# Belis0811/MaskUnet

Hardware: AMD Instinct MI355X
Metric: 128x128 images/sec (fwd+bwd) (higher is better)
Workload: dtype f16; 1 GPU; ADE20K-semantic shape 128x128, c_out=150, batch=64/GPU, 1-head MaskAttn-UNet fwd+bwd, train mode; global_batch=64, parallelism=dp1, mask_mode=fixed, loss=maskunet_amd.CrossEntropyLoss on module output, optimizer_in_step=False, hip_graph=False

## Files before the change

include/maskunet_hip.h:

```cpp
#ifndef MASKUNET_HIP_H
#define MASKUNET_HIP_H

#ifdef __cplusplus
extern "C" {
#endif

#define MU_OK 0
#define MU_ERR_ARG (-1)
#define MU_ERR_SHAPE (-2)
#define MU_ERR_LAUNCH (-3)
#define MU_ERR_WORKSPACE (-4)

#define MU_F32 0
#define MU_F16 1
#define MU_F32X 2

#define MU_ACT_NONE 0
#define MU_ACT_GELU 1
#define MU_ACT_RELU 2

const char* mu_version_host(void);

int mu_transpose(const void* src, int src_dtype, long src_ld, void* dst, int dst_dtype, long dst_ld, int batch, int R, int C,
                 void* stream);
// ... 51 lines not shown

long mu_bn_workspace_bytes(int C);
int mu_bn_train_stats(const void* x, long M, int C, long ld, float* mean, float* rstd, float* running_mean, float* running_var,
                      long* num_batches_tracked, int c_valid, float momentum, float eps, void* workspace, long ws_bytes, int dtype,
                      void* stream);
int mu_bn_train_stats_rows(const float* stat_part, int rows, long M, int C, float* mean, float* rstd, float* running_mean,
                           float* running_var, long* num_batches_tracked, int c_valid, float momentum, float eps, void* workspace,
                           long ws_bytes, void* stream);
int mu_bn_eval_stats(const float* running_mean, const float* running_var, float eps, float* mean, float* rstd, int C, int c_valid,
                     void* stream);
int mu_bn_eval_fold(const float* running_mean1, const float* running_var1, const float* gamma1, const float* beta1, float eps1,
                    const float* running_mean2, const float* running_var2, const float* gamma2, const float* beta2, float eps2,
                    const float* conv_bias, float* scale, float* shift, int C, int c_valid, void* stream);
int mu_bn_act_fwd(const void* x, const void* res, void* y, long M, int C, long ld, const float* mean, const float* rstd,
                  const float* gamma, const float* beta, int act, int dtype, void* stream);
int mu_bn_act_fwd_enc(const void* x, const void* res, void* y_enc, void* y16, long M, int C, const float* mean, const float* rstd,
                      const float* gamma, const float* beta, int act, void* stream);
int mu_bn_act_bwd(const void* x, const void* res, const void* grad_out, void* dx, void* dres, long M, int C, long ld,
                  const float* mean, const float* rstd, const float* gamma, const float* beta, int act, int training, float* dgamma,
                  float* dbeta, void* workspace, long ws_bytes, int dtype, void* stream);
int mu_bn_pair_compose(const float* rstd1, const float* gamma1, const float* beta1, const float* gamma2, int C, int c_valid, long M,
                       float eps1, float eps2, float momentum2, float* running_mean2, float* running_var2,
                       long* num_batches_tracked2, float* gamma_eff, float* xhat_scale, float* dgamma2_coef, float* dgamma1_coef,
                       void* stream);
int mu_bn_act_bwd_scaled(const void* x, const void* res, const void* grad_out, void* dx, void* dres, long M, int C, long ld,
                         const float* mean, const float* rstd, const float* gamma, const float* beta, int act, int training,
                         float* dgamma, float* dbeta, const float* xhat_scale, void* workspace, long ws_bytes, int dtype, void* stream);

int mu_bn_pair_bwd(const void* x, const void* grad_out, void* dx, long M, int C, long ld, const float* mean, const float* rstd,
                   const float* gamma_eff, const float* beta2, const float* xhat_scale, const float* dgamma2_coef,
                   const float* dgamma1_coef, float* pair_grads, float* dbeta2, void* workspace, long ws_bytes, int dtype, void* stream);

int mu_bn_act_bwd_h(const void* x, const void* res, const void* grad_out, void* dx_h, void* dres, long M, int C, const float* mean,
                    const float* rstd, const float* gamma, const float* beta, int act, int training, float* dgamma, float* dbeta,
                    float* dy_scale, void* workspace, long ws_bytes, void* stream);
int mu_bn_pair_bwd_h(const void* x, const void* grad_out, void* dx_h, long M, int C, const float* mean, const float* rstd,
                     const float* gamma_eff, const float* beta2, const float* xhat_scale, const float* dgamma2_coef,
                     const float* dgamma1_coef, float* pair_grads, float* dbeta2, float* dy_scale, void* workspace, long ws_bytes,
                     void* stream);

long mu_ln_sample_workspace_bytes(int B);
int mu_ln_sample_fwd(const void* x, const float* w, const float* b, void* y, float* mean, float* rstd, int B, long L, float eps,
                     void* workspace, long ws_bytes, int dtype, void* stream);
int mu_ln_sample_bwd(const void* x, const void* dy, const float* w, const float* mean, const float* rstd, void* dx, float* dw,
                     float* db, int B, long L, void* workspace, long ws_bytes, int dtype, void* stream);

int mu_maxpool2_fwd(const void* x, void* y, int B, int H, int W, int C, int dtype, void* stream);
int mu_maxpool2_bwd(const void* x, const void* dy, void* dx, int B, int H, int W, int C, int dtype, void* stream);
int mu_maxpool2_bwd_acc(const void* x, const void* dy, const void* dy2, const void* dx_add, void* dx, int B, int H, int W, int C, int dtype,
                        void* stream);
int mu_upcat_fwd(const void* x, const void* skip, void* y, int B, int h, int w, int Cx, int Cs, int dtype, void* stream);
int mu_upcat_bwd(const void* dy, void* dx, void* dskip, int B, int h, int w, int Cx, int Cs, int dtype, void* stream);
int mu_upcat_bwd_acc(const void* dy, const void* dy2, void* dx, void* dskip, int B, int h, int w, int Cx, int Cs, int dtype, void* stream);
int mu_upcat_compact_fwd(const void* x, const void* skip, void* y, int B, int h, int w, int Cx_ld, int Cx_valid, int Cs_ld, int Cs_valid,
                         int Ct_ld, int dtype, void* stream);
int mu_upcat_compact_bwd(const void* dy, void* dx, void* dskip, int B, int h, int w, int Cx_ld, int Cx_valid, int Cs_ld, int Cs_valid,
                         int Ct_ld, int dtype, void* stream);
int mu_dropout(const void* x, void* y, long n, float p, unsigned long long seed, const unsigned char* mask, unsigned char* mask_out,
               int dtype, void* stream);
int mu_dropout_step(const void* x, void* y, long n, float p, unsigned long long seed, const unsigned long long* seed_step,
// ... 145 lines not shown
```

maskunet_amd/_lib.py:

```python
from __future__ import annotations

import ctypes
import os
from ctypes import c_char_p, c_float, c_int, c_long, c_ulonglong, c_void_p

import torch

_HERE = os.path.dirname(os.path.abspath(__file__))
LIB_PATH = os.environ.get("MU_LIB_PATH") or os.path.join(_HERE, "libmaskunet_hip.so")

MU_F32, MU_F16, MU_F32X = 0, 1, 2
ACT_NONE, ACT_GELU, ACT_RELU = 0, 1, 2
MU_IDMAP_I32, MU_IDMAP_I64, MU_IDMAP_RGB8 = 0, 1, 2
_ERR = {-1: "MU_ERR_ARG", -2: "MU_ERR_SHAPE", -3: "MU_ERR_LAUNCH", -4: "MU_ERR_WORKSPACE"}

P, I, L, F = c_void_p, c_int, c_long, c_float
SIGNATURES = {
    "mu_version_host": (c_char_p, []),
    "mu_transpose": (I, [P, I, L, P, I, L, I, I, I, P]),
    "mu_transpose_pad": (I, [P, I, L, P, I, L, I, I, I, I, P]),
    "mu_cast": (I, [P, I, P, I, L, P]),
    "mu_split_encode": (I, [P, P, L, P]),
    "mu_split_encode_h": (I, [P, P, L, P]),
    "mu_split_encode_h4": (I, [P, P, L, P]),
# ... 25 lines not shown
    "mu_conv_wgrad_bias": (I, [P, P, P, P, I, I, I, I, I, I, I, I, L, L, P, L, I, P]),
    "mu_colsum_workspace_bytes": (L, [I]),
    "mu_colsum": (I, [P, L, I, L, P, P, L, I, P]),
    "mu_bn_workspace_bytes": (L, [I]),
    "mu_bn_train_stats": (I, [P, L, I, L, P, P, P, P, P, I, F, F, P, L, I, P]),
    "mu_bn_train_stats_rows": (I, [P, I, L, I, P, P, P, P, P, I, F, F, P, L, P]),
    "mu_bn_eval_stats": (I, [P, P, F, P, P, I, I, P]),
    "mu_bn_act_fwd": (I, [P, P, P, L, I, L, P, P, P, P, I, I, P]),
    "mu_bn_act_bwd": (I, [P, P, P, P, P, L, I, L, P, P, P, P, I, I, P, P, P, L, I, P]),
    "mu_bn_pair_compose": (I, [P, P, P, P, I, I, L, F, F, F, P, P, P, P, P, P, P, P]),
    "mu_bn_act_bwd_scaled": (I, [P, P, P, P, P, L, I, L, P, P, P, P, I, I, P, P, P, P, L, I, P]),
    "mu_bn_pair_bwd": (I, [P, P, P, L, I, L, P, P, P, P, P, P, P, P, P, P, L, I, P]),
    "mu_ln_sample_workspace_bytes": (L, [I]),
    "mu_ln_sample_fwd": (I, [P, P, P, P, P, P, I, L, F, P, L, I, P]),
    "mu_ln_sample_bwd": (I, [P, P, P, P, P, P, P, P, I, L, P, L, I, P]),
    "mu_maxpool2_fwd": (I, [P, P, I, I, I, I, I, P]),
    "mu_maxpool2_bwd": (I, [P, P, P, I, I, I, I, I, P]),
    "mu_upcat_fwd": (I, [P, P, P, I, I, I, I, I, I, P]),
    "mu_upcat_bwd": (I, [P, P, P, I, I, I, I, I, I, P]),
    "mu_upcat_compact_fwd": (I, [P, P, P, I, I, I, I, I, I, I, I, I, P]),
    "mu_upcat_compact_bwd": (I, [P, P, P, I, I, I, I, I, I, I, I, I, P]),
    "mu_dropout": (I, [P, P, L, F, c_ulonglong, P, P, I, P]),
    "mu_dropout_step": (I, [P, P, L, F, c_ulonglong, P, P, P, I, P]),
    "mu_add": (I, [P, P, P, L, I, P]),
    "mu_attn_fwd": (I, [P, P, P, P, P, P, P, P, P, P, P, I, I, I, I, F, I, P]),
    "mu_attn_bwd_workspace_bytes": (L, [I, I, I]),
    "mu_attn_bwd": (I, [P, P, P, P, P, P, P, P, P, P, P, P, P, P, P, I, I, I, I, P, L, I, P]),
    "mu_gather_rows": (I, [P, L, P, P, P, I, I, I, P]),
    "mu_scatter_rows": (I, [P, P, P, P, L, I, I, I, P]),
    "mu_softmax_rows": (I, [P, I, I, P, F, I, P]),
# ... 180 lines not shown
```

maskunet_amd/csrc/norm.hip:

```cpp
#include "common.h"
#include "../../include/maskunet_hip.h"

#define MU_STAT_MAXBLK 1024

template <typename T, int MODE, int ACT = -1, int RES = -1, bool MAXT = false>
__global__ __launch_bounds__(256, 1) void bn_partial_kernel(const T* __restrict__ x, const T* __restrict__ g, const T* __restrict__ res,
                                                         T* __restrict__ dzbuf, long M, int C, long ld,
                                                         const float* __restrict__ mean, const float* __restrict__ rstd,
                                                         const float* __restrict__ gamma, const float* __restrict__ beta, int act_arg,
                                                         double* __restrict__ part, float* __restrict__ pmax = nullptr) {
    constexpr int N = Vec16<T>::N;
    constexpr int U = MODE == 0 ? 8 : 2;
    constexpr bool FAST = sizeof(T) == 2;
    const int act = ACT >= 0 ? ACT : act_arg;
    const bool has_res = RES >= 0 ? (RES != 0) : (res != nullptr);
    extern __shared__ __attribute__((aligned(16))) double sh[];
    const int cv = C / N;
    const int rpi = 256 / cv;
    const int tc = threadIdx.x % cv, tr = threadIdx.x / cv;
    const long r0 = (long)blockIdx.x * (U * rpi), r1 = M;
    const long rstride = (long)gridDim.x * (U * rpi);
    double s0[N], s1[N];
    float mxg[N], mxx[N];
#pragma unroll
// ... 181 lines not shown
    if (lane) return;
    dbeta[c] = (float)a;
    dgamma[c] = (float)b;
    if (pair_grads) {
        pair_grads[c] = pc2[c] * (float)b;
        pair_grads[C + c] = pc1[c] * (float)b;
        pair_grads[2 * C + c] = 0.f;
    }
    const float s1c = training ? (float)(a / (double)M) : 0.f;
    const float s2c = training ? (float)((xscale ? (double)xscale[c] : 1.0) * b / (double)M) : 0.f;
    s1[c] = s1c;
    s2[c] = s2c;
    if (bound) bound[c] = fabsf(gamma[c] * rstd[c]) * (mg + fabsf(s1c) + mx * fabsf(s2c));
}

template <typename T, bool ENC = false, int ACT = -1, int RES = -1>
__global__ __launch_bounds__(256) void bn_act_fwd_kernel(const T* __restrict__ x, const T* __restrict__ res, T* __restrict__ y, long M,
                                                         int C, long ld, const float* __restrict__ mean, const float* __restrict__ rstd,
                                                         const float* __restrict__ gamma, const float* __restrict__ beta, int act_arg,
                                                         h16* __restrict__ y16 = nullptr) {
    constexpr int N = Vec16<T>::N;
    constexpr int U = 2;
    constexpr bool FAST = sizeof(T) == 2;
    const int act = ACT >= 0 ? ACT : act_arg;
    const bool has_res = RES >= 0 ? (RES != 0) : (res != nullptr);
    const int cv = C / N;
    const long total = M * cv;
    const long stride = (long)gridDim.x * 256;
    const long first = (long)blockIdx.x * 256 + threadIdx.x;
    const int c = (int)(first % cv) * N;
    const long rstep = stride / cv;
    float a[N], b[N];
#pragma unroll
    for (int i = 0; i < N; ++i) {
        a[i] = rstd[c + i] * gamma[c + i];
        b[i] = beta[c + i] - mean[c + i] * a[i];
    }
    for (long idx = first; idx < total; idx += U * stride) {
        const long r = idx / cv;
        Vec16<T> xv[U], rv[U];
#pragma unroll
        for (int u = 0; u < U; ++u) {
            if (idx + u * stride < total) {
                xv[u].load_nt(x + (r + u * rstep) * ld + c);
                if (has_res) rv[u].load_nt(res + (r + u * rstep) * ld + c);
            }
        }
#pragma unroll
        for (int u = 0; u < U; ++u) {
            if (idx + u * stride < total) {
                Vec16<T> o;
#pragma unroll
                for (int i = 0; i < N; i += 2) {
                    mu_f32x2 pp = __builtin_elementwise_fma(mu_f32x2{xv[u].get(i), xv[u].get(i + 1)}, mu_f32x2{a[i], a[i + 1]}, mu_f32x2{b[i], b[i + 1]});
                    if (has_res) pp += mu_f32x2{rv[u].get(i), rv[u].get(i + 1)};
                    float o0, o1;
                    mu_act2_t<FAST>(pp[0], pp[1], act, o0, o1);
                    o.set(i, o0);
                    o.set(i + 1, o1);
                }
                if constexpr (ENC) {
                    float o0 = o.get(0), o1 = o.get(1), o2 = o.get(2), o3 = o.get(3);
                    asm("" : "+v"(o0), "+v"(o1), "+v"(o2), "+v"(o3));
                    const uint4 e4 = mu_ench4((f32x4){o0, o1, o2, o3});
                    *reinterpret_cast<uint4*>(y + (r + u * rstep) * ld + c) = e4;
                    if (y16) *reinterpret_cast<uint2*>(y16 + (r + u * rstep) * (long)C + c) = make_uint2(e4.x, e4.y);
                } else {
                    o.store(y + (r + u * rstep) * ld + c);
                }
            }
        }
    }
}

template <typename T, bool RECOMP, bool ENC = false, int ACT = -1>
__global__ __launch_bounds__(256) void bn_bwd_apply_kernel(const T* __restrict__ x, const T* dzbuf, T* dx, long M, int C, long ld,
                                                           const float* __restrict__ mean, const float* __restrict__ rstd,
                                                           const float* __restrict__ gamma, const float* __restrict__ beta, int act_arg,
                                                           const float* __restrict__ s1, const float* __restrict__ s2,
                                                           const float* __restrict__ bound = nullptr, float* __restrict__ dy_scale = nullptr) {
    constexpr int N = Vec16<T>::N;
    constexpr int U = 2;
    constexpr bool FAST = sizeof(T) == 2;
    const int act = ACT >= 0 ? ACT : act_arg;
    const int cv = C / N;
    const long total = M * cv;
// ... 299 lines not shown
}

extern "C" int mu_bn_act_fwd(const void* x, const void* res, void* y, long M, int C, long ld, const float* mean, const float* rstd,
                             const float* gamma, const float* beta, int act, int dtype, void* stream) {
    if (!x || !y || !mean || !rstd || !gamma || !beta || M <= 0 || C <= 0 || C % 8 || ld < C) return MU_ERR_ARG;
    hipStream_t st = (hipStream_t)stream;
    if (act != MU_ACT_NONE && act != MU_ACT_GELU && act != MU_ACT_RELU) return MU_ERR_ARG;
    if (dtype == MU_F32X)
        return bn_act_fwd_launch<float, true>((const float*)x, (const float*)res, (float*)y, M, C, ld, mean, rstd, gamma, beta, act, st);
    return with_storage(dtype, [&](auto tag) -> int {
        using T = decltype(tag);
        return bn_act_fwd_launch<T, false>((const T*)x, (const T*)res, (T*)y, M, C, ld, mean, rstd, gamma, beta, act, st);
    });
}

template <typename T>
struct BnBwd {
    const T *x, *res, *g;
    T *dx, *dres;
    long M; int C; long ld;
    const float *mean, *rstd, *gamma, *beta;
    int act, training;
    float *dgamma, *dbeta;
    const float* xscale = nullptr;
    const float *pc2 = nullptr, *pc1 = nullptr;
    float* pair_grads = nullptr;
    float* dy_scale = nullptr;
};

template <typename T, bool ENC>
// ... 180 lines not shown
    double a = 0.0, c = 0.0;
    for (int k = lane; k < nchunk; k += 64) { a += part[((long)b * nchunk + k) * 2]; c += part[((long)b * nchunk + k) * 2 + 1]; }
    a = wave_sum_d(a); c = wave_sum_d(c);
    if (lane) return;
    if (mode == 0) {
        double m = a / (double)L, var = c / (double)L - m * m;
        if (var < 0.0) var = 0.0;
        o0[b] = (float)m;
        o1[b] = (float)(1.0 / sqrt(var + (double)eps));
    } else {
        o0[b] = (float)(a / (double)L);
        o1[b] = (float)(c / (double)L);
    }
}

template <typename T>
__global__ __launch_bounds__(256) void lns_fwd_apply_kernel(const T* __restrict__ x, const float* __restrict__ w, const float* __restrict__ bias,
                                                            const float* __restrict__ mean, const float* __restrict__ rstd, T* __restrict__ y,
                                                            long L, int B) {
    constexpr int N = Vec16<T>::N;
    const long nvec = L / N;
    for (long v = (long)blockIdx.x * 256 + threadIdx.x; v < nvec; v += (long)gridDim.x * 256) {
        float wv[N], bv[N];
#pragma unroll
        for (int i = 0; i < N; ++i) { wv[i] = w[v * N + i]; bv[i] = bias[v * N + i]; }
        for (int b = 0; b < B; ++b) {
            const float mu = mean[b], rs = rstd[b];
            Vec16<T> xv, o;
            xv.load_nt(x + (long)b * L + v * N);
#pragma unroll
            for (int i = 0; i < N; ++i) o.set(i, (xv.get(i) - mu) * rs * wv[i] + bv[i]);
            o.store(y + (long)b * L + v * N);
        }
    }
}

template <typename T>
__global__ __launch_bounds__(256) void lns_bwd_apply_kernel(const T* __restrict__ x, const T* __restrict__ dy, const float* __restrict__ w,
                                                            const float* __restrict__ mean, const float* __restrict__ rstd,
                                                            const float* __restrict__ m1, const float* __restrict__ m2, T* __restrict__ dx,
                                                            float* __restrict__ dw, float* __restrict__ db, long L, int B) {
    constexpr int N = Vec16<T>::N;
    const long nvec = L / N;
    for (long v = (long)blockIdx.x * 256 + threadIdx.x; v < nvec; v += (long)gridDim.x * 256) {
        float wv[N], aw[N], ab[N];
#pragma unroll
        for (int i = 0; i < N; ++i) { wv[i] = w[v * N + i]; aw[i] = 0.f; ab[i] = 0.f; }
        for (int b = 0; b < B; ++b) {
// ... 33 lines not shown
                                float eps, void* workspace, long ws_bytes, int dtype, void* stream) {
    if (!x || !w || !b || !y || !mean || !rstd || !workspace || B <= 0 || L <= 0 || L % 8) return MU_ERR_ARG;
    if (ws_bytes < LnWs::bytes(B)) return MU_ERR_WORKSPACE;
    hipStream_t st = (hipStream_t)stream;
    const LnWs ws(workspace, B);
    return with_storage(dtype, [&](auto tag) -> int {
        using T = decltype(tag);
        lns_partial_kernel<T, 0><<<dim3(LN_CHUNKS, B), 256, 0, st>>>((const T*)x, nullptr, nullptr, nullptr, nullptr, L, ws.part);
        lns_final_kernel<<<mu_cdiv(B, 4), 256, 0, st>>>(ws.part, LN_CHUNKS, L, eps, 0, mean, rstd, B);
        lns_fwd_apply_kernel<T><<<lns_apply_grid(L, Vec16<T>::N), 256, 0, st>>>((const T*)x, w, b, mean, rstd, (T*)y, L, B);
        MU_CHECK_LAUNCH();
        return MU_OK;
    });
}

extern "C" int mu_ln_sample_bwd(const void* x, const void* dy, const float* w, const float* mean, const float* rstd, void* dx,
                                float* dw, float* db, int B, long L, void* workspace, long ws_bytes, int dtype, void* stream) {
    if (!x || !dy || !w || !mean || !rstd || !dx || !dw || !db || !workspace || B <= 0 || L <= 0 || L % 8) return MU_ERR_ARG;
    if (ws_bytes < LnWs::bytes(B)) return MU_ERR_WORKSPACE;
    hipStream_t st = (hipStream_t)stream;
    const LnWs ws(workspace, B);
    return with_storage(dtype, [&](auto tag) -> int {
        using T = decltype(tag);
        lns_partial_kernel<T, 1><<<dim3(LN_CHUNKS, B), 256, 0, st>>>((const T*)x, (const T*)dy, w, mean, rstd, L, ws.part);
        lns_final_kernel<<<mu_cdiv(B, 4), 256, 0, st>>>(ws.part, LN_CHUNKS, L, 0.f, 1, ws.m1, ws.m2, B);
        lns_bwd_apply_kernel<T><<<lns_apply_grid(L, Vec16<T>::N), 256, 0, st>>>((const T*)x, (const T*)dy, w, mean, rstd, ws.m1, ws.m2, (T*)dx, dw, db, L, B);
        MU_CHECK_LAUNCH();
        return MU_OK;
    });
}
// ... 1 lines not shown
```

maskunet_amd/modules.py:

```python
from __future__ import annotations

import torch
import torch.nn as nn

from . import ops
from ._lib import ACT_GELU, ACT_NONE, ACT_RELU

_DEFAULT_DTYPE = torch.float32


def set_default_compute_dtype(dtype):
    global _DEFAULT_DTYPE
    if dtype not in (torch.float32, torch.float16):
        raise TypeError("compute dtype must be torch.float32 or torch.float16")
    _DEFAULT_DTYPE = dtype


class _HipModule(nn.Module):
    def __init__(self):
        super().__init__()
        self.compute_dtype = _DEFAULT_DTYPE

    def set_compute_dtype(self, dtype):
        if dtype not in (torch.float32, torch.float16):
# ... 167 lines not shown
    def forward_nhwc(self, x, skip_x, cx=None, cs=None, skip_link=None):
        link = ops.grad_link(x, skip_x)
        x = ops.upcat(x, skip_x, cx, cs, link, skip_link)
        return _conv_blocks(x, [self.conv[0], self.conv[1]], self.conv[2], link)

    def forward(self, x, skip_x):
        self._check_device(x)
        y = self.forward_nhwc(ops.to_nhwc(x, self.compute_dtype), ops.to_nhwc(skip_x, self.compute_dtype), x.shape[1], skip_x.shape[1])
        return ops.to_nchw(y, self.out_channels, x.dtype)


class _Head(nn.Sequential):
    """Conv2d 1x1 (bias) -> BatchNorm2d -> ReLU container with the reference's Sequential indices."""


def _head_1x1_bn_relu(seq, x):
    if ops.eval_fusable(seq[1]):
        return ops.conv_bn_act_eval(x, seq[0].weight, seq[0].bias, seq[1], ACT_RELU)
    y = ops.conv(x, seq[0].weight, seq[0].bias)
    return ops.bn_act(y, seq[1], ACT_RELU)


class UNet(_HipModule):

    def __init__(self, c_in=3, c_out=3, embed_dim=None, *, hw=128):
        super().__init__()
        self.c_out = c_out
        self.initial_conv = ConvBlock(c_in, 64)
        self.downsample1 = DownSample(64, 128)
        self.self_attention1 = Mask2FormerAttention(128, 128)
        self.downsample2 = DownSample(128, 256)
        self.self_attention2 = Mask2FormerAttention(256, 256)
        self.downsample3 = DownSample(256, 256)
        self.self_attention3 = Mask2FormerAttention(256, 256)

# ... 24 lines not shown

    def set_keep_masks(self, keeps):
        for blk, k in zip(self.attention_blocks(), keeps):
            blk.set_keep_mask(k)

    def set_mask_mode(self, mode):
        if mode not in ("fixed", "resample"):
            raise ValueError("mask_mode must be 'fixed' or 'resample'")
        for blk in self.attention_blocks():
            blk.mask_mode = mode

    def _drop(self, x, i):
        m = None if self.dropout_masks is None else self.dropout_masks[i]
        return ops.dropout(x, self.dropout.p, self.training, m)

    def forward_nhwc(self, x):
        if not (torch.is_grad_enabled() and self.training and ops.MULTI_PREP):
            return self._forward_nhwc(x)
        ws = self.__dict__.get("_conv_ws")
        if ws is None:
            ws = self.__dict__["_conv_ws"] = ([m for m in self.modules() if isinstance(m, nn.Conv2d)], {})
        weights = [m.weight for m in ws[0]]
        first = self.initial_conv.conv_block[0].weight
        ops.prep_conv_weights(ws[1], weights, x.dtype, fwd_only=() if x.requires_grad else (first,))
        try:
            return self._forward_nhwc(x)
        finally:
            for w in weights:
                w._mu_step = None

    def _forward_nhwc(self, x):
        x1 = self.initial_conv.forward_nhwc(x)
        l1 = ops.grad_link(x1)
        x2 = self.downsample1.forward_nhwc(x1, skip_link=l1)
        x2 = self.self_attention1.forward_nhwc(x2)
        l2 = ops.grad_link(x2)
        x3 = self.downsample2.forward_nhwc(x2, skip_link=l2)
        x3 = self.self_attention2.forward_nhwc(x3)
        l3 = ops.grad_link(x3)
        x4 = self.downsample3.forward_nhwc(x3, skip_link=l3)
        x4 = ops.cut_point(self.self_attention3.forward_nhwc(x4))

        x4 = _conv_blocks(x4, [self.bottom1, self.bottom2, self.bottom3])

        y = self.upsample1.forward_nhwc(x4, x3, skip_link=l3)
        y = self._drop(y, 0)
        y = self.self_attention4.forward_nhwc(y)
        y = self.upsample2.forward_nhwc(y, x2, skip_link=l2)
        y = self._drop(y, 1)
        y = self.self_attention5.forward_nhwc(y)
        y = self.upsample3.forward_nhwc(y, x1, skip_link=l1)
        B, H, W, _ = y.shape
        y = self.self_attention6.forward_nhwc(y, scramble=False)
        if tuple(self.norm.normalized_shape) != (64, H, W):
            raise RuntimeError(f"Given normalized_shape={list(self.norm.normalized_shape)}, expected input with shape "
                               f"[*, 64, {H}, {W}]")
        y = ops.ln_sample(y.view(B, -1), self.norm.weight, self.norm.bias, self.norm.eps)
        y = ops.to_nhwc(y.view(B, 64, H, W), self.compute_dtype)
        sem = _head_1x1_bn_relu(self.final_layer, y)
        if not self.three_head:
            return (sem,)
        emb = _head_1x1_bn_relu(self.embedding_head, y)
        bh = self.boundary_head
        if ops.eval_fusable(bh[1]):
            b = ops.conv_bn_act_eval(sem, bh[0].weight, bh[0].bias, bh[1], ACT_RELU)
        else:
            b = ops.conv(sem, bh[0].weight, bh[0].bias)
            b = ops.bn_act(b, bh[1], ACT_RELU)
        b = ops.conv(b, bh[3].weight, bh[3].bias)
        return sem, b, emb

    def logits_nhwc(self, x):
        self._check_device(x)
        return self.forward_nhwc(ops.to_nhwc(x, self.compute_dtype))[0]

    def forward_u8(self, images_u8_hwc, bgr=False, resample="cv2", check=False):
        if resample == "pil":
            from . import images as _images
            packed = _images.pack_images(images_u8_hwc)
            self._check_device(packed.data)
            H, W = int(self.norm.normalized_shape[1]), int(self.norm.normalized_shape[2])
            x, valid = _images.resize_pil_to_nhwc(packed, (H, W), self.compute_dtype, bgr=bgr)
            if check and not bool(valid.all()):
                raise RuntimeError(f"maskunet_amd: the Pillow resize refused images {(valid == 0).nonzero().flatten().tolist()} (size outside "
                                   "the contract: taller than 100 widths)")
            return self._finish(self.forward_nhwc(x))
        if resample != "cv2":
            raise ValueError(f'resample must be "cv2" or "pil", got {resample!r}')
        self._check_device(images_u8_hwc)
        H, W = int(self.norm.normalized_shape[1]), int(self.norm.normalized_shape[2])
        if tuple(images_u8_hwc.shape[1:3]) == (H, W) and not bgr:
            x = ops.u8_hwc_to_nhwc(images_u8_hwc, self.compute_dtype)
        else:
            x = ops.resize_u8_to_nhwc(images_u8_hwc, (W, H), self.compute_dtype, bgr=bgr)
        return self._finish(self.forward_nhwc(x))

    def forward(self, x):
        self._check_device(x)
        return self._finish(self.forward_nhwc(ops.to_nhwc(x, self.compute_dtype)))

    def _finish(self, outs):
        sem = ops.to_nchw(outs[0], self.c_out, torch.float32)
        if not self.three_head:
            return sem
        return sem, ops.to_nchw(outs[1], 1, torch.float32), ops.to_nchw(outs[2], self.embed_dim, torch.float32)


class InstanceUNet(UNet):

    def __init__(self, c_in=3, c_out=3, embed_dim=16, *, hw=128):
        super().__init__(c_in, c_out, embed_dim, hw=hw)


DoubleConv = ConvBlock
Down = DownSample
Up = UpSample
MaskAttention = Mask2FormerAttention


class OutConv(_HipModule):

    def __init__(self, in_channels, out_channels):
        super().__init__()
        self.final_layer = nn.Sequential(nn.Conv2d(in_channels, out_channels, kernel_size=1), nn.BatchNorm2d(out_channels), nn.ReLU())
        self.out_channels = out_channels

    def forward(self, x):
        self._check_device(x)
        y = _head_1x1_bn_relu(self.final_layer, ops.to_nhwc(x, self.compute_dtype))
        return ops.to_nchw(y, self.out_channels, x.dtype)
```

maskunet_amd/ops.py:

```python
from __future__ import annotations

import math
import os
from types import SimpleNamespace
from typing import NamedTuple

import torch
import torch.nn.functional as F
from torch.autograd.function import once_differentiable

from . import _lib
from ._lib import ACT_GELU, ACT_NONE, ACT_RELU, call, dt, mdt, ptr, stream, workspace


def pad32(c: int) -> int:
    return (c + 31) // 32 * 32


def _pad_vec(v, n, fill):
    v = v.detach().float()
    if v.numel() == n:
        return v.contiguous()
    return F.pad(v, (0, n - v.numel()), value=fill)

# ... 481 lines not shown


def _bn_train_stats(x, stats, bn, nbt, momentum, mean, rstd):
    C = x.shape[-1]
    M = x.numel() // C
    cv, rm, rv = bn.weight.numel(), bn.running_mean, bn.running_var
    ws = workspace(_lib.load().mu_bn_workspace_bytes(C), x.device)
    if stats is not None and stats.numel() > 0:
        call("mu_bn_train_stats_rows", ptr(stats), stats.shape[0], M, C, ptr(mean), ptr(rstd), ptr(rm), ptr(rv), ptr(nbt), cv,
             float(momentum), float(bn.eps), ptr(ws), ws.numel(), stream())
    else:
        call("mu_bn_train_stats", ptr(x), M, C, C, ptr(mean), ptr(rstd), ptr(rm), ptr(rv), ptr(nbt), cv, float(momentum), float(bn.eps),
             ptr(ws), ws.numel(), dt(x), stream())


def _bn_act_fwd(x, res, bn, act, stats=None, enc=False):
    x = x.contiguous()
    training = bn.training or bn.running_mean is None
    nbt = bn.num_batches_tracked if (bn.training and bn.num_batches_tracked is not None) else None
    if nbt is not None and (nbt.device != x.device or nbt.dtype != torch.int64):
        nbt.add_(1)
        nbt = None
    momentum = 0.1 if bn.momentum is None else bn.momentum
    C = x.shape[-1]
    M = x.numel() // C
    cv = bn.weight.numel()
    g_p, b_p = _pad_vec(bn.weight, C, 1.0), _pad_vec(bn.bias, C, 0.0)
    mean = torch.empty(C, dtype=torch.float32, device=x.device)
    rstd = torch.empty_like(mean)
    if training:
        _bn_train_stats(x, stats, bn, nbt, momentum, mean, rstd)
    else:
        call("mu_bn_eval_stats", ptr(bn.running_mean), ptr(bn.running_var), float(bn.eps), ptr(mean), ptr(rstd), C, cv, stream())
    y = torch.empty_like(x)
    if res is not None:
        res = res.contiguous()
    if enc:
        y16 = torch.empty(x.shape, dtype=torch.float16, device=x.device)
        call("mu_bn_act_fwd_enc", ptr(x), ptr(res), ptr(y), ptr(y16), M, C, ptr(mean), ptr(rstd), ptr(g_p), ptr(b_p), act, stream())
        y = _Enc3(y, y16)
    else:
        call("mu_bn_act_fwd", ptr(x), ptr(res), ptr(y), M, C, C, ptr(mean), ptr(rstd), ptr(g_p), ptr(b_p), act, dt(x), stream())
    return y, ((x, res, mean, rstd, g_p, b_p), (act, bool(training), cv))


def _dx_out(x, dx_h):
    if not dx_h:
        return torch.empty_like(x)
    return _DyH(torch.empty(x.shape, dtype=torch.float16, device=x.device), torch.empty(2, dtype=torch.float32, device=x.device))


def _bn_act_bwd(saved, gy, dx_h=False):
# ... 15 lines not shown
    return dx, dres, dgamma[:cv], dbeta[:cv]


class _BNAct(torch.autograd.Function):

    @staticmethod
    def forward(ctx, x, res, gamma, beta, bn, act, stats=None):
        y, (tensors, ctx.m) = _bn_act_fwd(x, res, bn, act, stats)
        ctx.save_for_backward(*tensors)
        return y

    @staticmethod
    @once_differentiable
    def backward(ctx, gy):
        return _bn_act_bwd((ctx.saved_tensors, ctx.m), gy) + (None, None, None)


BN_PAIR = os.environ.get("MU_BN_PAIR", "1") != "0"


def _bn_pair_ok(bn1, bn2, x):
    both_train = (bn1.training and bn2.training and bn1.running_mean is not None and bn2.running_mean is not None
                  and bn1.weight is not None and bn2.weight is not None)
    ok = both_train and BN_PAIR and all(t is not None and t.device == x.device and t.dtype == torch.int64
                                        for t in (bn1.num_batches_tracked, bn2.num_batches_tracked))
    return ok and bn1.momentum is not None and bn2.momentum is not None


def _bn_pair_fwd(x, bn1, bn2, stats=None):
    x = x.contiguous()
# ... 318 lines not shown
        x, wf, mean, rstd = ctx.saved_tensors
        gy = gy.contiguous()
        B = x.shape[0]
        L = x.numel() // B
        dx = torch.empty_like(x)
        dw = grad_out(ctx.wparam, (L,), x.device)
        db = grad_out(ctx.bparam, (L,), x.device)
        ws = workspace(_lib.load().mu_ln_sample_workspace_bytes(B), x.device)
        call("mu_ln_sample_bwd", ptr(x), ptr(gy), ptr(wf), ptr(mean), ptr(rstd), ptr(dx), ptr(dw), ptr(db), B, L, ptr(ws),
             ws.numel(), dt(x), stream())
        return dx, dw.view(ctx.wshape), db.view(ctx.wshape), None


def ln_sample(x, w, b, eps):
    return _LNSample.apply(x, w, b, eps)


def _transpose_tokens(src, R, C):
    B = src.shape[0]
    dst = torch.empty((B, C, R), dtype=src.dtype, device=src.device)
    call("mu_transpose", ptr(src), dt(src), C, ptr(dst), dt(dst), R, B, R, C, stream())
    return dst


def _pad_param(t, C):
    return F.pad(t.detach().float(), [p for n in reversed(t.shape) for p in (0, C - n)])


def _refuse_padded_scramble(scramble, cv, C):
    if scramble and cv != C:
# ... 249 lines not shown
```

Before: 2286 images/sec.

## Fuse NCHW output transpose into head BN-act and NHWC transpose into LayerNorm apply

Adds a BN+activation forward kernel that writes both the NHWC result and a transposed NCHW copy through a shared-memory tile, so the model's final heads no longer need a separate to_nchw pass. It also adds a LayerNorm-apply kernel that reads NCHW-flattened input and writes the padded NHWC layout directly, removing the separate to_nhwc conversion. The backward passes use explicit transposes to map gradients back to the original layouts. This trades two standalone layout-conversion kernels for more complex tiled kernels, and the backward adds its own transpose work.

```diff
diff --git a/include/maskunet_hip.h b/include/maskunet_hip.h
--- a/include/maskunet_hip.h
+++ b/include/maskunet_hip.h
@@ -89,6 +89,8 @@
                     const float* conv_bias, float* scale, float* shift, int C, int c_valid, void* stream);
 int mu_bn_act_fwd(const void* x, const void* res, void* y, long M, int C, long ld, const float* mean, const float* rstd,
                   const float* gamma, const float* beta, int act, int dtype, void* stream);
+int mu_bn_act_fwd_nchw(const void* x, void* y, void* y_nchw, int B, int HW, int C, int Cp, const float* mean, const float* rstd,
+                       const float* gamma, const float* beta, int act, int dtype, int out_dtype, void* stream);
 int mu_bn_act_fwd_enc(const void* x, const void* res, void* y_enc, void* y16, long M, int C, const float* mean, const float* rstd,
                       const float* gamma, const float* beta, int act, void* stream);
 int mu_bn_act_bwd(const void* x, const void* res, const void* grad_out, void* dx, void* dres, long M, int C, long ld,
@@ -119,6 +121,8 @@
                      void* workspace, long ws_bytes, int dtype, void* stream);
 int mu_ln_sample_bwd(const void* x, const void* dy, const float* w, const float* mean, const float* rstd, void* dx, float* dw,
                      float* db, int B, long L, void* workspace, long ws_bytes, int dtype, void* stream);
+int mu_ln_sample_fwd_nhwc(const void* x, const float* w, const float* b, void* y, float* mean, float* rstd, int B, int C, int HW, int Cp,
+                          float eps, void* workspace, long ws_bytes, int dtype, void* stream);
 
 int mu_maxpool2_fwd(const void* x, void* y, int B, int H, int W, int C, int dtype, void* stream);
 int mu_maxpool2_bwd(const void* x, const void* dy, void* dx, int B, int H, int W, int C, int dtype, void* stream);
diff --git a/maskunet_amd/_lib.py b/maskunet_amd/_lib.py
--- a/maskunet_amd/_lib.py
+++ b/maskunet_amd/_lib.py
@@ -63,6 +63,8 @@
     "mu_ln_sample_workspace_bytes": (L, [I]),
     "mu_ln_sample_fwd": (I, [P, P, P, P, P, P, I, L, F, P, L, I, P]),
     "mu_ln_sample_bwd": (I, [P, P, P, P, P, P, P, P, I, L, P, L, I, P]),
+    "mu_ln_sample_fwd_nhwc": (I, [P, P, P, P, P, P, I, I, I, I, F, P, L, I, P]),
+    "mu_bn_act_fwd_nchw": (I, [P, P, P, I, I, I, I, P, P, P, P, I, I, I, P]),
     "mu_maxpool2_fwd": (I, [P, P, I, I, I, I, I, P]),
     "mu_maxpool2_bwd": (I, [P, P, P, I, I, I, I, I, P]),
     "mu_upcat_fwd": (I, [P, P, P, I, I, I, I, I, I, P]),
diff --git a/maskunet_amd/csrc/norm.hip b/maskunet_amd/csrc/norm.hip
--- a/maskunet_amd/csrc/norm.hip
+++ b/maskunet_amd/csrc/norm.hip
@@ -219,6 +219,32 @@
     if (bound) bound[c] = fabsf(gamma[c] * rstd[c]) * (mg + fabsf(s1c) + mx * fabsf(s2c));
 }
 
+template <int N>
+__device__ __forceinline__ void bn_affine_coef(const float* __restrict__ mean, const float* __restrict__ rstd, const float* __restrict__ gamma,
+                                               const float* __restrict__ beta, int c, float (&a)[N], float (&b)[N]) {
+#pragma unroll
+    for (int i = 0; i < N; ++i) {
+        a[i] = rstd[c + i] * gamma[c + i];
+        b[i] = beta[c + i] - mean[c + i] * a[i];
+    }
+}
+template <typename T, bool FAST>
+__device__ __forceinline__ Vec16<T> bn_act_vec(const Vec16<T>& xv, const Vec16<T>& rv, bool has_res, const float (&a)[Vec16<T>::N],
+                                               const float (&b)[Vec16<T>::N], int act) {
+    constexpr int N = Vec16<T>::N;
+    Vec16<T> o;
+#pragma unroll
+    for (int i = 0; i < N; i += 2) {
+        mu_f32x2 pp = __builtin_elementwise_fma(mu_f32x2{xv.get(i), xv.get(i + 1)}, mu_f32x2{a[i], a[i + 1]}, mu_f32x2{b[i], b[i + 1]});
+        if (has_res) pp += mu_f32x2{rv.get(i), rv.get(i + 1)};
+        float o0, o1;
+        mu_act2_t<FAST>(pp[0], pp[1], act, o0, o1);
+        o.set(i, o0);
+        o.set(i + 1, o1);
+    }
+    return o;
+}
+
 template <typename T, bool ENC = false, int ACT = -1, int RES = -1>
 __global__ __launch_bounds__(256) void bn_act_fwd_kernel(const T* __restrict__ x, const T* __restrict__ res, T* __restrict__ y, long M,
                                                          int C, long ld, const float* __restrict__ mean, const float* __restrict__ rstd,
@@ -236,11 +262,7 @@
     const int c = (int)(first % cv) * N;
     const long rstep = stride / cv;
     float a[N], b[N];
-#pragma unroll
-    for (int i = 0; i < N; ++i) {
-        a[i] = rstd[c + i] * gamma[c + i];
-        b[i] = beta[c + i] - mean[c + i] * a[i];
-    }
+    bn_affine_coef<N>(mean, rstd, gamma, beta, c, a, b);
     for (long idx = first; idx < total; idx += U * stride) {
         const long r = idx / cv;
         Vec16<T> xv[U], rv[U];
@@ -254,16 +276,7 @@
 #pragma unroll
         for (int u = 0; u < U; ++u) {
             if (idx + u * stride < total) {
-                Vec16<T> o;
-#pragma unroll
-                for (int i = 0; i < N; i += 2) {
-                    mu_f32x2 pp = __builtin_elementwise_fma(mu_f32x2{xv[u].get(i), xv[u].get(i + 1)}, mu_f32x2{a[i], a[i + 1]}, mu_f32x2{b[i], b[i + 1]});
-                    if (has_res) pp += mu_f32x2{rv[u].get(i), rv[u].get(i + 1)};
-                    float o0, o1;
-                    mu_act2_t<FAST>(pp[0], pp[1], act, o0, o1);
-                    o.set(i, o0);
-                    o.set(i + 1, o1);
-                }
+                const Vec16<T> o = bn_act_vec<T, FAST>(xv[u], rv[u], has_res, a, b, act);
                 if constexpr (ENC) {
                     float o0 = o.get(0), o1 = o.get(1), o2 = o.get(2), o3 = o.get(3);
                     asm("" : "+v"(o0), "+v"(o1), "+v"(o2), "+v"(o3));
@@ -275,6 +288,67 @@
                 }
             }
         }
+    }
+}
+
+#define MU_NCHW_PT 4
+template <typename T> struct NV4 { T v[4]; };
+template <typename T, typename TD, int ACT>
+__global__ __launch_bounds__(256) void bn_act_fwd_nchw_kernel(const T* __restrict__ x, T* __restrict__ y, TD* __restrict__ out, int HW, int C,
+                                                              int Cp, const float* __restrict__ mean, const float* __restrict__ rstd,
+                                                              const float* __restrict__ gamma, const float* __restrict__ beta, bool ovec) {
+    constexpr int N = Vec16<T>::N;
+    constexpr int TPR = 64 / N;
+    constexpr int RPP = 256 / TPR;
+    constexpr int PASSES = 64 / RPP;
+    constexpr bool FAST = sizeof(T) == 2;
+    __shared__ float tile[2][64][65];
+    const int b = blockIdx.z, c0 = blockIdx.y * 64;
+    const int lc = (threadIdx.x % TPR) * N, lr = threadIdx.x / TPR;
+    const int c = c0 + lc;
+    const bool cok = c < Cp;
+    float a[N], bb[N];
+    if (cok) bn_affine_coef<N>(mean, rstd, gamma, beta, c, a, bb);
+    const T* xb = x + (long)b * HW * Cp;
+    T* yb = y + (long)b * HW * Cp;
+    TD* ob = out + (long)b * C * HW;
+    const int tv = (threadIdx.x & 15) * 4, ty = threadIdx.x >> 4;
+    int buf = 0;
+    for (int t = 0; t < MU_NCHW_PT; ++t) {
+        const int p0 = (blockIdx.x * MU_NCHW_PT + t) * 64;
+        if (p0 >= HW) break;
+        Vec16<T> xv[PASSES];
+#pragma unroll
+        for (int q = 0; q < PASSES; ++q) {
+            const int p = p0 + q * RPP + lr;
+            if (cok && p < HW) xv[q].load_nt(xb + (long)p * Cp + c);
+        }
+#pragma unroll
+        for (int q = 0; q < PASSES; ++q) {
+            const int r = q * RPP + lr, p = p0 + r;
+            if (cok && p < HW) {
+                const Vec16<T> o = bn_act_vec<T, FAST>(xv[q], xv[q], false, a, bb, ACT);
+                o.store(yb + (long)p * Cp + c);
+#pragma unroll
+                for (int i = 0; i < N; ++i) tile[buf][r][lc + i] = o.get(i);
+            }
+        }
+        __syncthreads();
+#pragma unroll
+        for (int i = ty; i < 64; i += 16) {
+            const int cc = c0 + i, p = p0 + tv;
+            if (cc >= C || p >= HW) continue;
+            NV4<TD> q;
+#pragma unroll
+            for (int k = 0; k < 4; ++k) q.v[k] = (TD)tile[buf][tv + k][i];
+            if (ovec && p + 3 < HW) {
+                *reinterpret_cast<NV4<TD>*>(ob + (long)cc * HW + p) = q;
+            } else {
+#pragma unroll
+                for (int k = 0; k < 4; ++k) if (p + k < HW) ob[(long)cc * HW + p + k] = q.v[k];
+            }
+        }
+        buf ^= 1;
     }
 }
 
@@ -604,6 +678,24 @@
     });
 }
 
+extern "C" int mu_bn_act_fwd_nchw(const void* x, void* y, void* y_nchw, int B, int HW, int C, int Cp, const float* mean, const float* rstd,
+                                  const float* gamma, const float* beta, int act, int dtype, int out_dtype, void* stream) {
+    if (!x || !y || !y_nchw || !mean || !rstd || !gamma || !beta || B <= 0 || HW <= 0 || C <= 0 || Cp < C || Cp % 8) return MU_ERR_ARG;
+    hipStream_t st = (hipStream_t)stream;
+    if (act != MU_ACT_NONE && act != MU_ACT_GELU && act != MU_ACT_RELU) return MU_ERR_ARG;
+    if (B > 65535) return MU_ERR_SHAPE;
+    return with_storage2(dtype, out_dtype, [&](auto stag, auto dtag) -> int {
+        using T = decltype(stag);
+        using TD = decltype(dtag);
+        const bool ovec = (size_t)y_nchw % (4 * sizeof(TD)) == 0 && HW % 4 == 0;
+        const dim3 grid(mu_cdiv(HW, 64 * MU_NCHW_PT), mu_cdiv(Cp, 64), B);
+        MU_BN_ACT_SWITCH(act, (bn_act_fwd_nchw_kernel<T, TD, A_><<<grid, 256, 0, st>>>((const T*)x, (T*)y, (TD*)y_nchw, HW, C, Cp, mean, rstd,
+                                                                                     gamma, beta, ovec)))
+        MU_CHECK_LAUNCH();
+        return MU_OK;
+    });
+}
+
 template <typename T>
 struct BnBwd {
     const T *x, *res, *g;
@@ -814,6 +906,8 @@
     }
 }
 
+__device__ __forceinline__ float lns_affine(float x, float mu, float rs, float w, float b) { return (x - mu) * rs * w + b; }
+
 template <typename T>
 __global__ __launch_bounds__(256) void lns_fwd_apply_kernel(const T* __restrict__ x, const float* __restrict__ w, const float* __restrict__ bias,
                                                             const float* __restrict__ mean, const float* __restrict__ rstd, T* __restrict__ y,
@@ -829,9 +923,82 @@
             Vec16<T> xv, o;
             xv.load_nt(x + (long)b * L + v * N);
 #pragma unroll
-            for (int i = 0; i < N; ++i) o.set(i, (xv.get(i) - mu) * rs * wv[i] + bv[i]);
+            for (int i = 0; i < N; ++i) o.set(i, lns_affine(xv.get(i), mu, rs, wv[i], bv[i]));
             o.store(y + (long)b * L + v * N);
         }
+    }
+}
+
+template <typename T>
+__global__ __launch_bounds__(256) void lns_fwd_apply_nhwc_kernel(const T* __restrict__ x, const float* __restrict__ w, const float* __restrict__ bias,
+                                                                 const float* __restrict__ mean, const float* __restrict__ rstd, T* __restrict__ y,
+                                                                 int C, int HW, int Cp, int B, int bper) {
+    constexpr int N = Vec16<T>::N;
+    constexpr int TPR = 64 / N;
+    constexpr int RPP = 256 / TPR;
+    constexpr int PASSES = 64 / RPP;
+    __shared__ float tile[2][64][65];
+    const int p0 = blockIdx.x * 64, c0 = blockIdx.y * 64;
+    const int b0 = blockIdx.z * bper, b1 = (b0 + bper < B ? b0 + bper : B);
+    const int lp = (threadIdx.x % TPR) * N, lc = threadIdx.x / TPR;
+    const bool vec = HW % N == 0;
+    const long L = (long)C * HW;
+    float wv[PASSES][N], bv[PASSES][N];
+#pragma unroll
+    for (int q = 0; q < PASSES; ++q) {
+        const int c = c0 + q * RPP + lc;
+#pragma unroll
+        for (int i = 0; i < N; ++i) {
+            const bool in = c < C && p0 + lp + i < HW;
+            wv[q][i] = in ? w[(long)c * HW + p0 + lp + i] : 0.f;
+            bv[q][i] = in ? bias[(long)c * HW + p0 + lp + i] : 0.f;
+        }
+    }
+    auto load_x = [&](int b, Vec16<T> (&xv)[PASSES]) {
+#pragma unroll
+        for (int q = 0; q < PASSES; ++q) {
+            const int c = c0 + q * RPP + lc;
+            const T* src = x + (long)b * L + (long)c * HW + p0 + lp;
+            xv[q].zero();
+            if (c >= C) continue;
+            if (vec) {
+                if (p0 + lp < HW) xv[q].load_nt(src);
+            } else {
+#pragma unroll
+                for (int i = 0; i < N; ++i) if (p0 + lp + i < HW) xv[q].set(i, (float)src[i]);
+            }
+        }
+    };
+    Vec16<T> nxt[PASSES];
+    if (b0 < b1) load_x(b0, nxt);
+    int buf = 0;
+    for (int b = b0; b < b1; ++b) {
+        Vec16<T> xv[PASSES];
+#pragma unroll
+        for (int q = 0; q < PASSES; ++q) xv[q] = nxt[q];
+        if (b + 1 < b1) load_x(b + 1, nxt);
+        const float mu = mean[b], rs = rstd[b];
+#pragma unroll
+        for (int q = 0; q < PASSES; ++q) {
+            const bool cin = c0 + q * RPP + lc < C;
+#pragma unroll
+            for (int i = 0; i < N; ++i)
+                tile[buf][lp + i][q * RPP + lc] = cin ? lns_affine(xv[q].get(i), mu, rs, wv[q][i], bv[q][i]) : 0.f;
+        }
+        __syncthreads();
+        T* yb = y + (long)b * HW * Cp;
+#pragma unroll
+        for (int q = 0; q < PASSES; ++q) {
+            const int idx = q * 256 + threadIdx.x;
+            const int px = idx / TPR, cv = (idx % TPR) * N;
+            if (p0 + px < HW && c0 + cv < Cp) {
+                Vec16<T> o;
+#pragma unroll
+                for (int i = 0; i < N; ++i) o.set(i, tile[buf][px][cv + i]);
+                o.store(yb + (long)(p0 + px) * Cp + c0 + cv);
+            }
+        }
+        buf ^= 1;
     }
 }
 
@@ -895,6 +1062,30 @@
     });
 }
 
+extern "C" int mu_ln_sample_fwd_nhwc(const void* x, const float* w, const float* b, void* y, float* mean, float* rstd, int B, int C, int HW,
+                                     int Cp, float eps, void* workspace, long ws_bytes, int dtype, void* stream) {
+    if (!x || !w || !b || !y || !mean || !rstd || !workspace || B <= 0 || C <= 0 || HW <= 0 || ((long)C * HW) % 8 || Cp < C || Cp % 8)
+        return MU_ERR_ARG;
+    if (ws_bytes < LnWs::bytes(B)) return MU_ERR_WORKSPACE;
+    hipStream_t st = (hipStream_t)stream;
+    const LnWs ws(workspace, B);
+    const long L = (long)C * HW;
+    const long tiles = (long)mu_cdiv(HW, 64) * mu_cdiv(Cp, 64);
+    long groups = (2048 + tiles - 1) / tiles;
+    groups = groups > B ? B : groups;
+    const int bper = mu_cdiv(B, groups);
+    const dim3 grid(mu_cdiv(HW, 64), mu_cdiv(Cp, 64), mu_cdiv(B, bper));
+    if (grid.y > 65535) return MU_ERR_SHAPE;
+    return with_storage(dtype, [&](auto tag) -> int {
+        using T = decltype(tag);
+        lns_partial_kernel<T, 0><<<dim3(LN_CHUNKS, B), 256, 0, st>>>((const T*)x, nullptr, nullptr, nullptr, nullptr, L, ws.part);
+        lns_final_kernel<<<mu_cdiv(B, 4), 256, 0, st>>>(ws.part, LN_CHUNKS, L, eps, 0, mean, rstd, B);
+        lns_fwd_apply_nhwc_kernel<T><<<grid, 256, 0, st>>>((const T*)x, w, b, mean, rstd, (T*)y, C, HW, Cp, B, bper);
+        MU_CHECK_LAUNCH();
+        return MU_OK;
+    });
+}
+
 extern "C" int mu_ln_sample_bwd(const void* x, const void* dy, const float* w, const float* mean, const float* rstd, void* dx,
                                 float* dw, float* db, int B, long L, void* workspace, long ws_bytes, int dtype, void* stream) {
     if (!x || !dy || !w || !mean || !rstd || !dx || !dw || !db || !workspace || B <= 0 || L <= 0 || L % 8) return MU_ERR_ARG;
diff --git a/maskunet_amd/modules.py b/maskunet_amd/modules.py
--- a/maskunet_amd/modules.py
+++ b/maskunet_amd/modules.py
@@ -205,11 +205,14 @@
     """Conv2d 1x1 (bias) -> BatchNorm2d -> ReLU container with the reference's Sequential indices."""
 
 
-def _head_1x1_bn_relu(seq, x):
+def _head_1x1_bn_relu(seq, x, nchw=None):
     if ops.eval_fusable(seq[1]):
-        return ops.conv_bn_act_eval(x, seq[0].weight, seq[0].bias, seq[1], ACT_RELU)
+        y = ops.conv_bn_act_eval(x, seq[0].weight, seq[0].bias, seq[1], ACT_RELU)
+        return y if nchw is None else (y, ops.to_nchw(y, *nchw))
     y = ops.conv(x, seq[0].weight, seq[0].bias)
-    return ops.bn_act(y, seq[1], ACT_RELU)
+    if nchw is None:
+        return ops.bn_act(y, seq[1], ACT_RELU)
+    return ops.bn_act_nchw(y, seq[1], ACT_RELU, *nchw)
 
 
 class UNet(_HipModule):
@@ -264,9 +267,9 @@
         m = None if self.dropout_masks is None else self.dropout_masks[i]
         return ops.dropout(x, self.dropout.p, self.training, m)
 
-    def forward_nhwc(self, x):
+    def forward_nhwc(self, x, finish=False):
         if not (torch.is_grad_enabled() and self.training and ops.MULTI_PREP):
-            return self._forward_nhwc(x)
+            return self._forward_nhwc(x, finish)
         ws = self.__dict__.get("_conv_ws")
         if ws is None:
             ws = self.__dict__["_conv_ws"] = ([m for m in self.modules() if isinstance(m, nn.Conv2d)], {})
@@ -274,12 +277,12 @@
         first = self.initial_conv.conv_block[0].weight
         ops.prep_conv_weights(ws[1], weights, x.dtype, fwd_only=() if x.requires_grad else (first,))
         try:
-            return self._forward_nhwc(x)
+            return self._forward_nhwc(x, finish)
         finally:
             for w in weights:
                 w._mu_step = None
 
-    def _forward_nhwc(self, x):
+    def _forward_nhwc(self, x, finish=False):
         x1 = self.initial_conv.forward_nhwc(x)
         l1 = ops.grad_link(x1)
         x2 = self.downsample1.forward_nhwc(x1, skip_link=l1)
@@ -305,12 +308,17 @@
         if tuple(self.norm.normalized_shape) != (64, H, W):
             raise RuntimeError(f"Given normalized_shape={list(self.norm.normalized_shape)}, expected input with shape "
                                f"[*, 64, {H}, {W}]")
-        y = ops.ln_sample(y.view(B, -1), self.norm.weight, self.norm.bias, self.norm.eps)
-        y = ops.to_nhwc(y.view(B, 64, H, W), self.compute_dtype)
-        sem = _head_1x1_bn_relu(self.final_layer, y)
+        if y.dtype == self.compute_dtype:
+            y = ops.ln_sample_nhwc(y.view(B, -1), self.norm.weight, self.norm.bias, self.norm.eps, 64, H, W)
+        else:
+            y = ops.ln_sample(y.view(B, -1), self.norm.weight, self.norm.bias, self.norm.eps)
+            y = ops.to_nhwc(y.view(B, 64, H, W), self.compute_dtype)
+        sem = _head_1x1_bn_relu(self.final_layer, y, (self.c_out, torch.float32) if finish else None)
         if not self.three_head:
-            return (sem,)
-        emb = _head_1x1_bn_relu(self.embedding_head, y)
+            return sem[1] if finish else (sem,)
+        emb = _head_1x1_bn_relu(self.embedding_head, y, (self.embed_dim, torch.float32) if finish else None)
+        if finish:
+            (sem, sem_out), (emb, emb_out) = sem, emb
         bh = self.boundary_head
         if ops.eval_fusable(bh[1]):
             b = ops.conv_bn_act_eval(sem, bh[0].weight, bh[0].bias, bh[1], ACT_RELU)
@@ -318,6 +326,8 @@
             b = ops.conv(sem, bh[0].weight, bh[0].bias)
             b = ops.bn_act(b, bh[1], ACT_RELU)
         b = ops.conv(b, bh[3].weight, bh[3].bias)
+        if finish:
+            return sem_out, ops.to_nchw(b, 1, torch.float32), emb_out
         return sem, b, emb
 
     def logits_nhwc(self, x):
@@ -334,7 +344,7 @@
             if check and not bool(valid.all()):
                 raise RuntimeError(f"maskunet_amd: the Pillow resize refused images {(valid == 0).nonzero().flatten().tolist()} (size outside "
                                    "the contract: taller than 100 widths)")
-            return self._finish(self.forward_nhwc(x))
+            return self.forward_nhwc(x, finish=True)
         if resample != "cv2":
             raise ValueError(f'resample must be "cv2" or "pil", got {resample!r}')
         self._check_device(images_u8_hwc)
@@ -343,11 +353,11 @@
             x = ops.u8_hwc_to_nhwc(images_u8_hwc, self.compute_dtype)
         else:
             x = ops.resize_u8_to_nhwc(images_u8_hwc, (W, H), self.compute_dtype, bgr=bgr)
-        return self._finish(self.forward_nhwc(x))
-
-    def forward(self, x):
-        self._check_device(x)
-        return self._finish(self.forward_nhwc(ops.to_nhwc(x, self.compute_dtype)))
+        return self.forward_nhwc(x, finish=True)
+
+    def forward(self, x):
+        self._check_device(x)
+        return self.forward_nhwc(ops.to_nhwc(x, self.compute_dtype), finish=True)
 
     def _finish(self, outs):
         sem = ops.to_nchw(outs[0], self.c_out, torch.float32)
@@ -377,5 +387,4 @@
 
     def forward(self, x):
         self._check_device(x)
-        y = _head_1x1_bn_relu(self.final_layer, ops.to_nhwc(x, self.compute_dtype))
-        return ops.to_nchw(y, self.out_channels, x.dtype)
+        return _head_1x1_bn_relu(self.final_layer, ops.to_nhwc(x, self.compute_dtype), (self.out_channels, x.dtype))[1]
diff --git a/maskunet_amd/ops.py b/maskunet_amd/ops.py
--- a/maskunet_amd/ops.py
+++ b/maskunet_amd/ops.py
@@ -519,7 +519,7 @@
              ptr(ws), ws.numel(), dt(x), stream())
 
 
-def _bn_act_fwd(x, res, bn, act, stats=None, enc=False):
+def _bn_act_fwd(x, res, bn, act, stats=None, enc=False, nchw=None):
     x = x.contiguous()
     training = bn.training or bn.running_mean is None
     nbt = bn.num_batches_tracked if (bn.training and bn.num_batches_tracked is not None) else None
@@ -540,7 +540,14 @@
     y = torch.empty_like(x)
     if res is not None:
         res = res.contiguous()
-    if enc:
+    if nchw is not None:
+        cn, out_dtype = nchw
+        B, H, W = x.shape[:3]
+        y_nchw = torch.empty((B, cn, H, W), dtype=out_dtype, device=x.device)
+        call("mu_bn_act_fwd_nchw", ptr(x), ptr(y), ptr(y_nchw), B, H * W, cn, C, ptr(mean), ptr(rstd), ptr(g_p), ptr(b_p), act, dt(x),
+             dt(y_nchw), stream())
+        y = (y, y_nchw)
+    elif enc:
         y16 = torch.empty(x.shape, dtype=torch.float16, device=x.device)
         call("mu_bn_act_fwd_enc", ptr(x), ptr(res), ptr(y), ptr(y16), M, C, ptr(mean), ptr(rstd), ptr(g_p), ptr(b_p), act, stream())
         y = _Enc3(y, y16)
@@ -586,6 +593,35 @@
     @once_differentiable
     def backward(ctx, gy):
         return _bn_act_bwd((ctx.saved_tensors, ctx.m), gy) + (None, None, None)
+
+
+class _BNActNCHW(torch.autograd.Function):
+
+    @staticmethod
+    def forward(ctx, x, gamma, beta, bn, act, cn, out_dtype):
+        (y, y_nchw), (tensors, ctx.m) = _bn_act_fwd(x, None, bn, act, nchw=(cn, out_dtype))
+        ctx.save_for_backward(*tensors)
+        ctx.set_materialize_grads(False)
+        return y, y_nchw
+
+    @staticmethod
+    @once_differentiable
+    def backward(ctx, gy, gn):
+        x = ctx.saved_tensors[0]
+        if gn is not None:
+            gn = gn.contiguous()
+            B, cn, H, W = gn.shape
+            t = torch.empty_like(x)
+            call("mu_transpose_pad", ptr(gn), dt(gn), H * W, ptr(t), dt(t), x.shape[-1], B, cn, H * W, x.shape[-1], stream())
+            gy = t if gy is None else gy + t
+        dx, _, dgamma, dbeta = _bn_act_bwd((ctx.saved_tensors, ctx.m), gy)
+        return dx, dgamma, dbeta, None, None, None, None
+
+
+def bn_act_nchw(x, bn, act, cn, out_dtype=torch.float32):
+    y, y_nchw = _BNActNCHW.apply(x, bn.weight, bn.bias, bn, act, cn, out_dtype)
+    y_nchw._mu_nhwc = (y, cn, y_nchw._version)
+    return y, y_nchw
 
 
 BN_PAIR = os.environ.get("MU_BN_PAIR", "1") != "0"
@@ -934,6 +970,48 @@
 
 def ln_sample(x, w, b, eps):
     return _LNSample.apply(x, w, b, eps)
+
+
+class _LNSampleNHWC(torch.autograd.Function):
+
+    @staticmethod
+    def forward(ctx, x, w, b, eps, C, H, W):
+        x = x.contiguous()
+        B = x.shape[0]
+        Cp = pad32(C)
+        wf, bf = w.detach().float().contiguous().view(-1), b.detach().float().contiguous().view(-1)
+        y = torch.empty((B, H, W, Cp), dtype=x.dtype, device=x.device)
+        mean = torch.empty(B, dtype=torch.float32, device=x.device)
+        rstd = torch.empty_like(mean)
+        ws = workspace(_lib.load().mu_ln_sample_workspace_bytes(B), x.device)
+        call("mu_ln_sample_fwd_nhwc", ptr(x), ptr(wf), ptr(bf), ptr(y), ptr(mean), ptr(rstd), B, C, H * W, Cp, float(eps), ptr(ws),
+             ws.numel(), dt(x), stream())
+        ctx.save_for_backward(x, wf, mean, rstd)
+        ctx.wshape, ctx.chw = tuple(w.shape), (C, H, W)
+        ctx.wparam, ctx.bparam = w, b
+        return y
+
+    @staticmethod
+    @once_differentiable
+    def backward(ctx, gy):
+        x, wf, mean, rstd = ctx.saved_tensors
+        C, H, W = ctx.chw
+        gy = gy.contiguous()
+        B, Cp = x.shape[0], gy.shape[-1]
+        L = C * H * W
+        g = torch.empty((B, L), dtype=x.dtype, device=x.device)
+        call("mu_transpose", ptr(gy), dt(gy), Cp, ptr(g), dt(g), H * W, B, H * W, C, stream())
+        dx = torch.empty_like(x)
+        dw = grad_out(ctx.wparam, (L,), x.device)
+        db = grad_out(ctx.bparam, (L,), x.device)
+        ws = workspace(_lib.load().mu_ln_sample_workspace_bytes(B), x.device)
+        call("mu_ln_sample_bwd", ptr(x), ptr(g), ptr(wf), ptr(mean), ptr(rstd), ptr(dx), ptr(dw), ptr(db), B, L, ptr(ws),
+             ws.numel(), dt(x), stream())
+        return dx, dw.view(ctx.wshape), db.view(ctx.wshape), None, None, None, None
+
+
+def ln_sample_nhwc(x, w, b, eps, C, H, W):
+    return _LNSampleNHWC.apply(x, w, b, eps, C, H, W)
 
 
 def _transpose_tokens(src, R, C):
```

Result: no change. 2286 images/sec (median of 2 runs) (+0.0%).
